# vibhaska/delta

Measured on AMD Instinct MI355X. Metric: log actions replayed/sec + achieved HBM GB/s, 1/2/4/8 GPU, 10M-file table, higher is better.
Workload: dtype u8/int64; 1 GPU; config 3: 10M-file checkpoint + 30 JSON commits, 16000032 actions -> 10000000 live files, 30% remove/re-add churn, retention cutoff; actions=16000032, json_bytes=1775145997, checkpoint_bytes=859787616, parallelism=single GPU

## Files before the change

### delta_amd/csrc/json_lane.h

```cpp
#pragma once
#include <cstdint>
#include <cstring>

#if defined(__HIPCC__)
#define JL_HD __host__ __device__ __forceinline__
#define JL_UNROLL _Pragma("unroll")
#else
#define JL_HD inline
#define JL_UNROLL
#endif

namespace dr {
namespace jl {

enum : uint8_t { K_NONE = 0, K_ADD = 1, K_REMOVE = 2, K_METADATA = 3, K_TXN = 4, K_PROTOCOL = 5, K_CDC = 6,
                 K_COMMITINFO = 7, K_ERROR = 15 };
enum : uint8_t { F_HAS_DELTS = 1, F_PATH_ESCAPED = 4, F_PATH_NULL = 8 };

struct LineOut {
  uint8_t kind;
  uint8_t flags;
  uint8_t hard;
  uint32_t path_off;
  uint32_t path_len;
  int64_t size;
  int64_t delts;
};

JL_HD uint32_t zbytes(uint32_t y) { return ~(((y & 0x7F7F7F7Fu) + 0x7F7F7F7Fu) | y | 0x7F7F7F7Fu); }
JL_HD uint32_t lt20(uint32_t x) { return ~((x | 0x80808080u) - 0x20202020u) & ~x & 0x80808080u; }
JL_HD uint32_t gather4(uint32_t m) {
  m >>= 7;
  m |= m >> 7;
  m |= m >> 14;
  return m & 0xFu;
}
JL_HD uint32_t prefix_xor16(uint32_t x) {
  x ^= x << 1;
  x ^= x << 2;
  x ^= x << 4;
  x ^= x << 8;
  return x & 0xFFFFu;
}

struct Win {
  uint32_t q, bs, st, sp, ctrl;
};

JL_HD uint32_t perm_b32(uint32_t s0, uint32_t s1, uint32_t sel) {
#if defined(__HIP_DEVICE_COMPILE__)
  return __builtin_amdgcn_perm(s0, s1, sel);
#else
  uint32_t r = 0;
  for (int k = 0; k < 4; ++k) {
    const uint32_t b = (sel >> (8 * k)) & 0xFFu;
    const uint32_t v = b < 4 ? (s1 >> (8 * b)) & 0xFFu : b < 8 ? (s0 >> (8 * (b - 4))) & 0xFFu : b == 0x0C ? 0u : 0xFFu;
    r |= v << (8 * k);
  }
  return r;
#endif
}
constexpr uint32_t CLS_LO0 = 0x40414048u, CLS_LO1 = 0x40404040u, CLS_LO2 = 0x44504040u, CLS_LO3 = 0x40404462u;
constexpr uint32_t CLS_HI0 = 0x10294040u, CLS_HI1 = 0x04000600u;
JL_HD uint32_t class_bytes(uint32_t x) {
  const uint32_t lo = x & 0x0F0F0F0Fu;
  const uint32_t sel = lo & 0x07070707u;
  const uint32_t a = perm_b32(CLS_LO1, CLS_LO0, sel), b = perm_b32(CLS_LO3, CLS_LO2, sel);
  const uint32_t m8 = perm_b32(0u, 0u, ((lo >> 3) & 0x01010101u) | 0x0C0C0C0Cu);
  const uint32_t tlo = (m8 & b) | (~m8 & a);
  const uint32_t thi = perm_b32(CLS_HI1, CLS_HI0, (x >> 4) & 0x07070707u);
  const uint32_t neg = perm_b32(0u, 0u, ((x >> 7) & 0x01010101u) | 0x0C0C0C0Cu);
  return tlo & thi & ~neg;
}
JL_HD uint32_t gather_bit(uint32_t r, int c) {
  uint32_t m = (r >> c) & 0x01010101u;
  m |= m >> 7;
  m |= m >> 14;
  return m & 0xFu;
}
JL_HD uint32_t delta_swap(uint32_t y, uint32_t delta, uint32_t mask) {
  const uint32_t t = (y ^ (y >> delta)) & mask;
  return y ^ t ^ (t << delta);
}

JL_HD void classify(const uint32_t w[4], Win& m) {
  uint32_t r[4], nib[4];
#if defined(__HIP_DEVICE_COMPILE__)
#pragma unroll
#endif
  for (int d = 0; d < 4; ++d) {
    r[d] = class_bytes(w[d]);
    nib[d] = (r[d] & 0x0F0F0F0Fu) | (((r[d] >> 2) | (r[d] >> 3)) & 0x04040404u);
  }
  uint32_t y0 = nib[0] | (nib[1] << 4), y1 = nib[2] | (nib[3] << 4);
  y0 = delta_swap(delta_swap(y0, 7, 0x00AA00AAu), 14, 0x0000CCCCu);
  y1 = delta_swap(delta_swap(y1, 7, 0x00AA00AAu), 14, 0x0000CCCCu);
  const uint32_t qb = perm_b32(y1, y0, 0x05010400u), ss = perm_b32(y1, y0, 0x07030602u);
  m.q = qb & 0xFFFFu;
  m.bs = qb >> 16;
  m.st = ss & 0xFFFFu;
  m.sp = ss >> 16;
  m.ctrl = 0;
  if ((r[0] | r[1] | r[2] | r[3]) & 0x40404040u)
    for (int d = 0; d < 4; ++d) m.ctrl |= gather_bit(r[d], 6) << (4 * d);
}

JL_HD uint32_t win_byte(const uint32_t w[4], uint32_t k) {
  const uint32_t d = k >> 2;
  const uint32_t x = d == 0 ? w[0] : d == 1 ? w[1] : d == 2 ? w[2] : w[3];
  return (x >> (8 * (k & 3))) & 0xFFu;
}

JL_HD uint32_t ctz32(uint32_t x) {
#if defined(__HIP_DEVICE_COMPILE__)
  return uint32_t(__builtin_ctz(x));
#else
  return uint32_t(__builtin_ctz(x));
#endif
}
JL_HD uint32_t popc32(uint32_t x) { return uint32_t(__builtin_popcount(x)); }

enum : uint8_t { SC_BAD = 0, SC_NULL, SC_TRUE, SC_FALSE, SC_INT, SC_NUM };

JL_HD bool key_eq(const uint8_t* s, uint32_t n, const char* k, uint32_t kn) {
  if (n != kn) return false;
  for (uint32_t i = 0; i < n; ++i)
    if (s[i] != uint8_t(k[i])) return false;
  return true;
}
JL_HD uint8_t action_key(const uint8_t* s, uint32_t n) {
  switch (n) {
    case 3:
      if (key_eq(s, n, "add", 3)) return K_ADD;
      if (key_eq(s, n, "txn", 3)) return K_TXN;
      if (key_eq(s, n, "cdc", 3)) return K_CDC;
      return 0;
    case 6: return key_eq(s, n, "remove", 6) ? K_REMOVE : 0;
    case 8:
      if (key_eq(s, n, "metaData", 8)) return K_METADATA;
      if (key_eq(s, n, "protocol", 8)) return K_PROTOCOL;
      return 0;
    case 10: return key_eq(s, n, "commitInfo", 10) ? K_COMMITINFO : 0;
    default: return 0;
  }
}
enum : uint8_t { FK_OTHER = 0, FK_PATH, FK_SIZE, FK_DELTS };
JL_HD uint8_t file_key(const uint8_t* s, uint32_t n) {
  if (n == 4) {
    if (key_eq(s, n, "path", 4)) return FK_PATH;
    if (key_eq(s, n, "size", 4)) return FK_SIZE;
    return FK_OTHER;
  }
  if (n == 17 && key_eq(s, n, "deletionTimestamp", 17)) return FK_DELTS;
  return FK_OTHER;
}

enum : uint32_t { T_OBJ_OPEN = 0, T_ARR_OPEN, T_OBJ_CLOSE, T_ARR_CLOSE, T_COLON, T_COMMA, T_STR_OPEN,
                  T_STR_CLOSE, T_STR_CLOSE_ESC, T_SCALAR, T_STRING, T_STRING_ESC, T_SCALAR_LONG = 13 };
enum : uint32_t { TF_COLON = 0x10u, TF_COMMA = 0x20u, TF_MASK = 0x30u };
constexpr uint32_t TOK_MAX_LINE = 65535;
constexpr uint32_t TOK_MAX_SCALAR = 4095;
constexpr uint32_t TOK_MAX_AUX = 1023;
// ... 433 lines not shown
    }
    d.state = S_AFTER;
  }
}

template <bool General>
JL_HD void dfa_token_own(const uint8_t* p, uint32_t tok, Dfa<General>& d) {
  const uint32_t cls = tok_cls(tok), off = tok_off(tok);
  const uint8_t stt = d.state;
  if (cls == T_STRING || cls == T_STRING_ESC) {
    if (dfa_str_open(off, d)) dfa_str_close(p, off + 1 + tok_aux(tok), cls == T_STRING_ESC, d);
    return;
  }
  if (cls == T_STR_OPEN) {
    dfa_str_open(off, d);
    return;
  }
  if (cls == T_STR_CLOSE || cls == T_STR_CLOSE_ESC) {
    dfa_str_close(p, off, cls == T_STR_CLOSE_ESC, d);
    return;
  }
  if (cls == T_SCALAR || cls == T_SCALAR_LONG) {
    if (!(stt == S_VALUE || stt == S_ARR_FIRST)) { d.status = ST_BAD; return; }
    const uint32_t L = cls == T_SCALAR ? tok_aux(tok) : tok_long_len(tok);
    int64_t v = 0;
    const uint8_t sc = scalar_fast(p + off, L, &v);
    if (sc == SC_BAD) { d.status = ST_BAD; return; }
    d.sc_checked += L;
    if (d.depth == 1) {
      if (sc == SC_NULL) {
        if (d.k1) d.present &= ~(1u << d.k1);
        if (d.k1 == K_ADD) d.fadd = FileObj{0, 0, 0, 0, F_PATH_NULL};
        if (d.k1 == K_REMOVE) d.frm = FileObj{0, 0, 0, 0, F_PATH_NULL};
      } else {
        if (d.k1 == K_ADD || d.k1 == K_REMOVE) { d.status = ST_BAD; return; }
        if (d.k1) d.present |= 1u << d.k1;
      }
    } else if (d.depth == 2 && d.in_file) {
      if (d.k2 == FK_PATH) {
        if (sc != SC_NULL) { d.status = ST_BAD; return; }
        d.cur.path_off = 0;
        d.cur.path_len = 0;
        d.cur.flags = uint8_t((d.cur.flags & ~F_PATH_ESCAPED) | F_PATH_NULL);
      } else if (d.k2 == FK_SIZE) {
        if (sc == SC_NULL) d.cur.size = 0;
        else if (sc == SC_INT) d.cur.size = v;
        else { d.status = ST_BAD; return; }
      } else if (d.k2 == FK_DELTS) {
        if (sc == SC_NULL) { d.cur.delts = 0; d.cur.flags &= ~F_HAS_DELTS; }
        else if (sc == SC_INT) { d.cur.delts = v; d.cur.flags |= F_HAS_DELTS; }
        else { d.status = ST_BAD; return; }
      }
    }
    d.state = S_AFTER;
    return;
  }
  if (cls == T_COLON) {
    if (stt != S_COLON) { d.status = ST_BAD; return; }
    d.state = S_VALUE;
    return;
  }
  if (cls == T_COMMA) {
    if (stt != S_AFTER || d.depth == 0) { d.status = ST_BAD; return; }
    d.state = d.is_arr(d.depth) ? S_VALUE : S_KEY;
    return;
  }
  if (cls == T_OBJ_OPEN || cls == T_ARR_OPEN) {
    const bool arr = cls == T_ARR_OPEN;
    if (!(stt == S_VALUE || stt == S_ARR_FIRST || (stt == S_START && !arr))) { d.status = ST_BAD; return; }
    if (d.depth == 2 && d.in_file && d.k2 != FK_OTHER) { d.status = ST_BAD; return; }
    if (d.depth == 1 && (d.k1 == K_ADD || d.k1 == K_REMOVE)) {
      if (arr) { d.status = ST_BAD; return; }
      d.in_file = true;
      d.k2 = FK_OTHER;
      d.cur = FileObj{0, 0, 0, 0, F_PATH_NULL};
    }
    if (d.depth >= 62) {
      if (!General) { d.status = ST_HARD; return; }
      if (d.depth + 1 >= GEN_MAX_DEPTH) { d.status = ST_BAD; return; }
    }
    ++d.depth;
    d.set_arr(d.depth, arr);
    d.state = arr ? S_ARR_FIRST : S_OBJ_FIRST;
    return;
  }
  {
    const bool arr = cls == T_ARR_CLOSE;
    if (d.depth == 0) { d.status = ST_BAD; return; }
    const bool top_arr = d.is_arr(d.depth);
    if (arr != top_arr || !(stt == S_AFTER || stt == (arr ? S_ARR_FIRST : S_OBJ_FIRST))) { d.status = ST_BAD; return; }
    if (d.depth == 2) {
      if (d.in_file) {
        const bool ad = d.k1 == K_ADD;
        d.fadd.path_off = ad ? d.cur.path_off : d.fadd.path_off;
        d.fadd.path_len = ad ? d.cur.path_len : d.fadd.path_len;
        d.fadd.size = ad ? d.cur.size : d.fadd.size;
        d.fadd.delts = ad ? d.cur.delts : d.fadd.delts;
        d.fadd.flags = ad ? d.cur.flags : d.fadd.flags;
        d.frm.path_off = ad ? d.frm.path_off : d.cur.path_off;
        d.frm.path_len = ad ? d.frm.path_len : d.cur.path_len;
        d.frm.size = ad ? d.frm.size : d.cur.size;
        d.frm.delts = ad ? d.frm.delts : d.cur.delts;
        d.frm.flags = ad ? d.frm.flags : d.cur.flags;
        d.in_file = false;
      }
      if (d.k1) d.present |= 1u << d.k1;
    }
    --d.depth;
    d.state = d.depth == 0 ? S_DONE : S_AFTER;
  }
}

template <bool General>
JL_HD void dfa_token(const uint8_t* p, uint32_t tok, Dfa<General>& d) {
  dfa_token_own<General>(p, tok, d);
  const uint32_t fl = tok_flags(tok);
  if (fl == 0 || d.status != ST_OK) return;
  const bool colon = (fl & TF_COLON) != 0;
  const bool ok = fl != TF_MASK && (colon ? d.state == S_COLON : (d.state == S_AFTER && d.depth != 0));
  if (!ok) { d.status = ST_BAD; return; }
  d.state = (colon || d.is_arr(d.depth)) ? S_VALUE : S_KEY;
}

template <bool General>
JL_HD void dfa_finish(const Tokenizer& tz, const Dfa<General>& d, LineOut& out) {
  out.kind = K_NONE;
  out.flags = 0;
  out.hard = 0;
  out.path_off = 0;
  out.path_len = 0;
  out.size = 0;
  out.delts = 0;
  if (tz.status == ST_HARD || d.status == ST_HARD) { out.hard = 1; return; }
  if (tz.status == ST_OK && d.status == ST_OK && d.state == S_START && tz.sc_bytes == 0) return;
  if (tz.status != ST_OK || d.status != ST_OK || d.state != S_DONE || tz.sc_bytes != d.sc_checked) {
    out.kind = K_ERROR;
    return;
  }
  const uint32_t pr = d.present;
  out.kind = (pr & (1u << K_ADD)) ? K_ADD : (pr & (1u << K_REMOVE)) ? K_REMOVE
           : (pr & (1u << K_METADATA)) ? K_METADATA : (pr & (1u << K_TXN)) ? K_TXN
           : (pr & (1u << K_PROTOCOL)) ? K_PROTOCOL : (pr & (1u << K_CDC)) ? K_CDC
           : (pr & (1u << K_COMMITINFO)) ? K_COMMITINFO : K_NONE;
  if (out.kind == K_ADD || out.kind == K_REMOVE) {
    const bool ad = out.kind == K_ADD;
    out.flags = ad ? d.fadd.flags : d.frm.flags;
    out.path_off = ad ? d.fadd.path_off : d.frm.path_off;
    out.path_len = ad ? d.fadd.path_len : d.frm.path_len;
    out.size = ad ? d.fadd.size : d.frm.size;
    out.delts = ad ? d.fadd.delts : d.frm.delts;
  }
}

template <bool General>
JL_HD void parse_line_t(const uint8_t* p, uint32_t n, LineOut& out) {
  Tokenizer tz;
  Dfa<General> d;
  if (n > TOK_MAX_LINE) {
    if (!General) { out = LineOut{0, 0, 1, 0, 0, 0, 0}; return; }
  }
  const uintptr_t pa = reinterpret_cast<uintptr_t>(p);
  const uint8_t* base = p - (pa & 15u);
  const uint32_t o0 = uint32_t(pa & 15);
  const uint32_t nwin = (o0 + n + 15) >> 4;
  auto step = [&](uint32_t t) {
    if (d.status == ST_OK) dfa_token<General>(p, t, d);
  };
  for (uint32_t j = 0; j < nwin && tz.status == ST_OK && d.status == ST_OK; ++j) {
    uint32_t w[4];
    load_window(base + 16u * j, w);
    tokenize_window<General>(p, n, w, int32_t(16u * j) - int32_t(o0), tz, step);
  }
  tokenize_end(n, tz, step);
  dfa_finish<General>(tz, d, out);
}

JL_HD void parse_line(const uint8_t* p, uint32_t n, LineOut& out) { parse_line_t<false>(p, n, out); }
JL_HD void parse_line_general(const uint8_t* p, uint32_t n, LineOut& out) { parse_line_t<true>(p, n, out); }

}
}
```

### delta_amd/csrc/k_json.hip

```cpp
#include <cstdlib>
#include <type_traits>

#include "dev_common.h"
#include "kernels.h"
#include "json_lane.h"
#include "canon.h"
#include "wave.h"
#include "ix_dev.h"

namespace dr {
namespace dev {

#ifdef DR_BOUNDS_CHECK
__device__ unsigned int dr_lds_bounds_hits;
#define DR_LDS_CHECK(ok, site, idx, lim)                                                                       \
  do {                                                                                                       \
    if (!(ok) && atomicAdd(&dr_lds_bounds_hits, 1u) < 32u)                                                   \
      printf("LDS-BOUNDS %s: index %llu, extent %llu (block %u thread %u)\n", site, (unsigned long long)(idx), \
             (unsigned long long)(lim), blockIdx.x, threadIdx.x);                                           \
  } while (0)
#else
#define DR_LDS_CHECK(ok, site, idx, lim) \
  do {                                   \
  } while (0)
// ... 14 lines not shown
template <typename Put>
__device__ __forceinline__ uint32_t block_newlines(const uint8_t* __restrict__ buf, uint64_t len, uint64_t blk,
                                                   Put put) {
  __shared__ uint32_t wsum[JSON_THREADS / 64];
  const uint32_t rel0 = threadIdx.x * JSON_BYTES_PER_THREAD;
  const uint64_t base = blk * JSON_BYTES_PER_BLOCK + rel0;
  uint32_t words[16];
  uint32_t c = 0;
  const bool full = base + JSON_BYTES_PER_THREAD <= len;
  if (full) {
    const uint4* p = reinterpret_cast<const uint4*>(buf + base);
#pragma unroll
    for (int i = 0; i < 4; ++i) {
      uint4 v = p[i];
      words[4 * i] = v.x; words[4 * i + 1] = v.y; words[4 * i + 2] = v.z; words[4 * i + 3] = v.w;
    }
#pragma unroll
    for (int i = 0; i < 16; ++i) c += count_nl_word(words[i]);
  } else {
    for (uint64_t i = base; i < len; ++i) c += buf[i] == '\n';
  }
  const int lane = threadIdx.x & 63, wv = threadIdx.x >> 6;
  uint32_t incl = c;
  for (int o = 1; o < 64; o <<= 1) {
    uint32_t t = __shfl_up(incl, o, 64);
    if (lane >= o) incl += t;
  }
  if (lane == 63) wsum[wv] = incl;
  __syncthreads();
  uint32_t woff = 0, total = 0;
  for (int i = 0; i < JSON_THREADS / 64; ++i) {
    woff += i < wv ? wsum[i] : 0u;
    total += wsum[i];
  }
  uint32_t r = woff + incl - c;
  if (full) {
#pragma unroll
    for (int i = 0; i < 16; ++i) {
      uint32_t t = nl_bytes(words[i]);
      while (t) {
        put(r++, rel0 + 4 * i + (__builtin_ctz(t) >> 3));
        t &= t - 1;
      }
    }
  } else {
    for (uint64_t i = base; i < len; ++i)
      if (buf[i] == '\n') put(r++, uint32_t(i - blk * JSON_BYTES_PER_BLOCK));
  }
  return total;
}

__global__ void __launch_bounds__(JSON_THREADS) k_json_index(const uint8_t* __restrict__ buf, uint64_t len,
                                                            uint32_t* __restrict__ block_counts,
                                                            uint16_t* __restrict__ slots) {
  uint16_t* slot = slots + uint64_t(blockIdx.x) * JSON_SLOT;
  const uint32_t total = block_newlines(buf, len, blockIdx.x, [&](uint32_t r, uint32_t pos) {
    if (r < uint32_t(JSON_SLOT)) slot[r] = uint16_t(pos);
  });
  if (threadIdx.x == 0) block_counts[blockIdx.x] = total;
}

__global__ void __launch_bounds__(JSON_THREADS) k_json_index1(const uint8_t* __restrict__ buf, uint64_t len,
                                                             uint64_t* __restrict__ nl, uint64_t* __restrict__ off2,
                                                             uint64_t* __restrict__ zero, uint32_t nzero) {
  if (threadIdx.x < nzero) zero[threadIdx.x] = 0;
  const uint32_t total = block_newlines(buf, len, 0, [&](uint32_t r, uint32_t pos) { nl[r] = pos; });
  if (threadIdx.x == 0) {
    off2[0] = 0;
    off2[1] = total;
  }
}

__global__ void __launch_bounds__(JSON_THREADS) k_json_place(const uint8_t* __restrict__ buf, uint64_t len,
                                                            const uint32_t* __restrict__ block_counts,
                                                            const uint64_t* __restrict__ block_off,
                                                            const uint16_t* __restrict__ slots,
                                                            uint64_t* __restrict__ nl) {
  const uint32_t cnt = block_counts[blockIdx.x];
  const uint64_t base = uint64_t(blockIdx.x) * JSON_BYTES_PER_BLOCK;
  uint64_t* out = nl + block_off[blockIdx.x];
  if (cnt <= uint32_t(JSON_SLOT)) {
    const uint16_t* slot = slots + uint64_t(blockIdx.x) * JSON_SLOT;
    for (uint32_t k = threadIdx.x; k < cnt; k += JSON_THREADS) out[k] = base + slot[k];
  } else {
    block_newlines(buf, len, blockIdx.x, [&](uint32_t r, uint32_t pos) { out[r] = base + pos; });
  }
}

constexpr int JL_T = 64;

__device__ __forceinline__ void emit_line(const JsonParseArgs& a, uint64_t line, uint64_t b, uint32_t n,
                                          const uint8_t* lp, const uint8_t* gp, const jl::LineOut& o) {
  const uint64_t idx = a.base + line;
  uint8_t flags = 0;
  uint64_t key = 0, path = 0;
  uint32_t plen = 0;
  int64_t size = 0, delts = 0;
  const uint8_t kind = o.kind;
  if (kind == K_ADD || kind == K_REMOVE) {
    flags = o.flags;
    path = reinterpret_cast<uint64_t>(gp + o.path_off);
    plen = o.path_len;
    size = o.size;
    delts = o.delts;
    if (!(flags & F_PATH_NULL)) {
      if ((flags & F_PATH_ESCAPED) || path_is_special(lp + o.path_off, plen)) {
        flags |= F_SPECIAL_PATH;
        atomicAdd(reinterpret_cast<unsigned long long*>(a.special_count), 1ull);
        atomicAdd(reinterpret_cast<unsigned long long*>(a.special_bytes), (unsigned long long)(plen + 8));
      } else {
        key = path_key(lp + o.path_off, plen);
      }
    } else {
      path = 0;
      plen = 0;
    }
  } else if (kind == K_METADATA || kind == K_TXN || kind == K_PROTOCOL) {
    const unsigned long long slot = atomicAdd(reinterpret_cast<unsigned long long*>(a.nonfile_count), 1ull);
    if (slot < a.nonfile_cap) {
      a.nonfile_idx[2 * slot] = line;
      a.nonfile_idx[2 * slot + 1] = b;
    }
  } else if (kind == K_ERROR) {
    atomicAdd(reinterpret_cast<unsigned long long*>(a.error_count), 1ull);
  }
  a.kind[idx] = kind;
  a.flags[idx] = flags;
  a.key[idx] = key;
  a.path_ptr[idx] = path;
  a.path_len[idx] = plen;
  if (a.path_ref) a.path_ref[idx] = pack_ref(path, plen);
  a.size[idx] = size;
  a.delts[idx] = delts;
  a.src_off[idx] = b;
  a.src_len[idx] = n;
}

#ifndef DR_JL_TOKCAP
#define DR_JL_TOKCAP 40
#endif
constexpr int JL_TOKCAP = DR_JL_TOKCAP;
#ifndef DR_JL_FLUSH
#define DR_JL_FLUSH (DR_JL_TOKCAP - 18)
#endif
static_assert(DR_JL_FLUSH >= 0 && DR_JL_FLUSH + 18 <= DR_JL_TOKCAP, "a window's tokens must fit behind the flush mark");
constexpr int JL_FLUSH = DR_JL_FLUSH;

#ifndef DR_JL_BATCH
#define DR_JL_BATCH 2
#endif
#ifndef DR_JL_WAVES
#define DR_JL_WAVES 1
#endif
constexpr uint32_t JL_SMALL_LINES = 256;
constexpr uint32_t JL_STAGE_BYTES = 24u * 1024u;

template <bool InlineHard = false>
__device__ __forceinline__ void walk_line(const JsonParseArgs& a, uint32_t* tokbuf, uint32_t lane, uint64_t line,
                                          bool live, uint64_t b, uint32_t n, const uint8_t* p) {
  jl::Tokenizer tz;
  jl::Dfa<false> d;
  if (!live) tz.status = jl::ST_BAD;
  else if (n > jl::TOK_MAX_LINE) tz.status = jl::ST_HARD;
  const uint32_t o0 = uint32_t(b & 15);
  const uint8_t* base = p - o0;
  const uint32_t nwin = tz.status == jl::ST_OK ? (o0 + n + 15) >> 4 : 0;
  uint32_t nt = 0;
#if DR_JL_BATCH > 1
  uint4 batch[DR_JL_BATCH];
#endif
  auto push = [&](uint32_t t) {
    DR_LDS_CHECK(nt < uint32_t(JL_TOKCAP), "walk_line tokbuf", nt, JL_TOKCAP);
    tokbuf[nt * JL_T + lane] = t;
    ++nt;
  };
  for (uint32_t j = 0;; ++j) {
    if (j < nwin && tz.status == jl::ST_OK) {
      uint32_t w[4];
#if DR_JL_BATCH > 1
      if (j % DR_JL_BATCH == 0) {
        const uint4* q = reinterpret_cast<const uint4*>(base + 16u * j);
#pragma unroll
        for (int k = 0; k < DR_JL_BATCH; ++k) batch[k] = j + k < nwin ? q[k] : make_uint4(0, 0, 0, 0);
      }
      uint4 v0 = batch[0];
#pragma unroll
      for (int k = 1; k < DR_JL_BATCH; ++k)
        if (j % DR_JL_BATCH == uint32_t(k)) v0 = batch[k];
      w[0] = v0.x; w[1] = v0.y; w[2] = v0.z; w[3] = v0.w;
#else
      jl::load_window(base + 16u * j, w);
#endif
      jl::tokenize_window<false>(p, n, w, int32_t(16u * j) - int32_t(o0), tz, push);
      if (j + 1 == nwin) jl::tokenize_end(n, tz, push);
    }
    const bool more = j + 1 < nwin && tz.status == jl::ST_OK;
    const bool anymore = __ballot(more) != 0ull;
    if (!anymore || __ballot(nt > uint32_t(JL_FLUSH)) != 0ull) {
      uint32_t mx = nt;
      for (int o = 32; o > 0; o >>= 1) mx = max(mx, uint32_t(__shfl_xor(int(mx), o, 64)));
#if !defined(DR_JL_EXP)
      for (uint32_t t = 0; t < mx; ++t)
        if (t < nt && d.status == jl::ST_OK) jl::dfa_token<false>(p, tokbuf[t * JL_T + lane], d);
#endif
      nt = 0;
    }
    if (!anymore) break;
  }
  if (!live) return;
  jl::LineOut o;
  jl::dfa_finish<false>(tz, d, o);
  if (o.hard) {
    if constexpr (InlineHard) {
      const uint8_t* gp = a.buf + b;
      jl::parse_line_general(gp, n, o);
      emit_line(a, line, b, n, gp, gp, o);
    } else {
      const unsigned long long k = atomicAdd(a.hard_count, 1ull);
      a.hard_idx[k] = line;
    }
    return;
  }
  emit_line(a, line, b, n, p, a.buf + b, o);
}

constexpr uint32_t T_NL = 12;
constexpr uint32_t TAPE_CAP = 4096;

constexpr uint64_t STRUCT_CLS = (uint64_t(jl::T_COLON) << 40) | (uint64_t(jl::T_OBJ_OPEN) << 44) |
                                (uint64_t(jl::T_COMMA) << 48) | (uint64_t(jl::T_OBJ_CLOSE) << 52);

__device__ __forceinline__ uint32_t escape16(uint32_t bs, uint32_t cin, uint32_t* cout) {
  const uint32_t bsn = bs & ~cin;
  const uint32_t follows = ((bsn << 1) | cin) & 0xFFFFu;
  const uint32_t odd_starts = bsn & ~0x5555u & ~follows;
  const uint32_t sum = odd_starts + bsn;
  *cout = (sum >> 16) & 1u;
  return (0x5555u ^ ((sum << 1) & 0xFFFFu)) & follows;
}

__device__ __forceinline__ uint64_t lanes_below() { return (1ull << wv::lane_id()) - 1ull; }

__device__ __forceinline__ void wave_sync() {
  __builtin_amdgcn_fence(__ATOMIC_RELEASE, "wavefront");
  __builtin_amdgcn_wave_barrier();
  __builtin_amdgcn_fence(__ATOMIC_ACQUIRE, "wavefront");
}

__device__ __forceinline__ int32_t from_lower(bool has, int32_t v, int32_t dflt) {
  constexpr uint32_t NONE = 0x80000000u;
  uint32_t x = has ? uint32_t(v) : NONE;
  x = wv::scan_incl(x, NONE, [](uint32_t e, uint32_t l) { return l == NONE ? e : l; });
  x = wv::shr1(x, NONE);
  return x == NONE ? dflt : int32_t(x);
}

template <uint32_t TCap, uint32_t NL, uint32_t SW>
__device__ __forceinline__ bool build_tape(const uint4* stage, uint32_t rb, uint32_t R, uint32_t nlines, uint32_t* tape,
                           uint16_t* nltok, uint8_t* tline, unsigned long long* phase = nullptr) {
  const uint32_t lane = wv::lane_id();
  DR_LDS_CHECK(uint64_t(rb) + R + 48 <= uint64_t(SW) * 16, "build_tape region", uint64_t(rb) + R + 48, SW * 16);
  if (uint64_t(rb) + R + 48 > uint64_t(SW) * 16) return false;
  const uint32_t a0 = rb & ~15u;
  const uint32_t skew = rb - a0;
  const uint32_t total = skew + R;
  const uint32_t nsteps = (total + 1023u) >> 10;
  uint32_t esc_c = 0, instr_c = 0, sc_c = 0, tbase = 0, nlc = 0;
  int32_t open_c = -1, bs_c = -1;
  for (uint32_t s = 0; s < nsteps; ++s) {
    const uint64_t ts0 = phase ? __builtin_amdgcn_s_memtime() : 0;
    const uint32_t wpos = (s << 10) + (lane << 4);
    const int32_t lo = int32_t(wpos) - int32_t(skew);
    DR_LDS_CHECK(wpos >= total || ((a0 + wpos) >> 4) < SW, "build_tape stage", (a0 + wpos) >> 4, SW);
    const uint4 v = stage[min((a0 + wpos) >> 4, SW - 1)];
    const uint32_t keep = wpos < total ? ~0u : 0u;
    const uint32_t w[4] = {v.x & keep, v.y & keep, v.z & keep, v.w & keep};
    const uint32_t vlo = lo < 0 ? (0xFFFFu << uint32_t(min(-lo, 16))) & 0xFFFFu : 0xFFFFu;
    const int32_t rem = int32_t(R) - lo;
    const uint32_t vhi = rem >= 16 ? 0xFFFFu : rem <= 0 ? 0u : (1u << uint32_t(rem)) - 1u;
    const uint32_t valid = vlo & vhi;
    jl::Win m;
    jl::classify(w, m);
    m.q &= valid; m.bs &= valid; m.st &= valid; m.sp &= valid; m.ctrl &= valid;
    uint32_t nl = 0;
#pragma unroll
    for (int d = 0; d < 4; ++d) nl |= jl::gather4(jl::zbytes(w[d] ^ 0x0a0a0a0au)) << (4 * d);
    nl &= valid;
    uint32_t c0;
    escape16(m.bs, 0u, &c0);
    const bool allbs = m.bs == 0xFFFFu;
    const uint32_t cin = uint32_t(from_lower(!allbs, int32_t(c0), int32_t(esc_c)));
    uint32_t cout;
    const uint32_t escaped = escape16(m.bs, cin, &cout);
    esc_c = uint32_t(__builtin_amdgcn_readlane(int(allbs ? cin : cout), 63));
    const uint32_t quote = m.q & ~escaped;
    const unsigned long long par = __ballot(__builtin_popcount(quote) & 1);
    const uint32_t sin = instr_c ^ uint32_t(__popcll(par & lanes_below()) & 1);
    const uint32_t instr = jl::prefix_xor16(quote) ^ (sin ? 0xFFFFu : 0u);
    instr_c ^= uint32_t(__popcll(par) & 1);
    bool bad = (m.ctrl & ~(nl & ~instr)) != 0 || (m.sp & ~instr) != 0;
    uint32_t oddesc = escaped & ~(m.q | m.bs) & valid;
    while (oddesc) {
      const uint32_t k = jl::ctz32(oddesc);
      oddesc &= oddesc - 1;
      const uint32_t c = jl::win_byte(w, k);
      bad |= !(c == '/' || c == 'b' || c == 'f' || c == 'n' || c == 'r' || c == 't');
    }
    const uint32_t st = m.st & ~instr;
    const uint32_t sc = valid & ~instr & ~quote & ~st & ~m.sp & ~m.ctrl;
    const uint32_t sc_prev = wv::shr1(sc >> 15, sc_c) & 1u;
    const uint32_t sc_begin = sc & ~(((sc << 1) | sc_prev) & 0xFFFFu);
    sc_c = uint32_t(__builtin_amdgcn_readlane(int(sc >> 15), 63)) & 1u;
    const uint32_t open = quote & instr, close = quote & ~instr;
    const uint32_t bsin = m.bs & instr;
    const int32_t last_open = open ? lo + 31 - __builtin_clz(open) : -1;
    const int32_t last_bs = bsin ? lo + 31 - __builtin_clz(bsin) : -1;
    const int32_t open_in = from_lower(open != 0, last_open, open_c);
    const int32_t bs_in = from_lower(bsin != 0, last_bs, bs_c);
    open_c = __builtin_amdgcn_readlane(open ? last_open : open_in, 63);
    bs_c = __builtin_amdgcn_readlane(bsin ? last_bs : bs_in, 63);
    const uint32_t tm = st | close | sc_begin | nl;
    const uint32_t cnt = uint32_t(__builtin_popcount(tm)) | (uint32_t(__builtin_popcount(nl)) << 16);
    const uint32_t incl = wv::scan_incl(cnt, 0u, [](uint32_t e, uint32_t l) { return e + l; });
    const uint32_t tot = uint32_t(__builtin_amdgcn_readlane(int(incl), 63));
    if (__ballot(bad)) return false;
    if (tbase + (tot & 0xFFFFu) > TCap || nlc + (tot >> 16) > NL) return false;
    uint32_t idx = tbase + ((incl - cnt) & 0xFFFFu);
    uint32_t nlr = nlc + ((incl - cnt) >> 16);
    bool longstr = false;
    const uint64_t ts1 = phase ? __builtin_amdgcn_s_memtime() : 0;
    uint32_t t = tm;
    const uint64_t wlo = uint64_t(w[0]) | (uint64_t(w[1]) << 32), whi = uint64_t(w[2]) | (uint64_t(w[3]) << 32);
    while (t) {
      const uint32_t k = jl::ctz32(t);
      t &= t - 1;
      const uint32_t bit = 1u << k, below = bit - 1u;
      const uint32_t pos = uint32_t(lo + int32_t(k));
      const uint32_t ob = open & below, bb = bsin & below;
      const int32_t op = ob ? lo + 31 - __builtin_clz(ob) : open_in;
      const int32_t lb = bb ? lo + 31 - __builtin_clz(bb) : bs_in;
      const uint32_t blen = pos - uint32_t(op) - 1u;
      const uint32_t c = uint32_t(((k & 8u) ? whi : wlo) >> ((k & 7u) * 8u)) & 0xFFu;
      const uint32_t lo4 = c & 15u;
      const uint32_t scls = uint32_t((STRUCT_CLS >> (4u * lo4)) & 15u) + (((0x2800u >> lo4) & ~(c >> 5)) & 1u);
      const bool isclose = (close & bit) != 0;
      longstr |= isclose & (blen >= 4096u);
      const uint32_t stok = (uint32_t(op) << 16) | ((blen & 0xFFFu) << 4) | (lb > op ? jl::T_STRING_ESC : jl::T_STRING);
      const uint32_t otok = (pos << 16) | ((st & bit) ? scls : (sc_begin & bit) ? jl::T_SCALAR : T_NL);
      DR_LDS_CHECK(idx < TCap, "build_tape tape", idx, TCap);
      DR_LDS_CHECK(nlr < NL || !(nl & bit), "build_tape nltok", nlr, NL);
      tline[idx] = uint8_t(nlr);
      const bool isnl = (nl & bit) != 0;
      nltok[isnl ? nlr : NL] = uint16_t(idx);
      nlr += isnl ? 1u : 0u;
      tape[idx++] = isclose ? stok : otok;
    }
    if (phase && lane == 0) {
      atomicAdd(&phase[6], (unsigned long long)(ts1 - ts0));
      atomicAdd(&phase[7], (unsigned long long)(__builtin_amdgcn_s_memtime() - ts1));
    }
    if (__ballot(longstr)) return false;
    tbase += tot & 0xFFFFu;
    nlc += tot >> 16;
  }
// ... 70 lines not shown
       : (L == 5 && w0[0] == 0x736C6166u && (w0[1] & 0xFFu) == 0x65u) ? jl::SC_FALSE
       : (isint && fits) ? jl::SC_INT : jl::SC_BAD;
}

template <uint32_t TCap, uint32_t NL>
__device__ __forceinline__ void tape_lines(const JsonParseArgs& a, uint64_t line0, uint32_t nlines, const uint8_t* sp,
                                           uint32_t sp_ext, uint64_t gb, const uint32_t* tape, const uint16_t* nltok,
                                           const uint8_t* tline, TapeAgg<NL>& g) {
  (void)sp_ext;
  const uint32_t lane = wv::lane_id();
  const uint64_t tw0 = a.phase ? __builtin_amdgcn_s_memtime() : 0;
  if (lane < NL) {
#pragma unroll
    for (int k = 0; k < 8; ++k) {
      g.mem[lane][k] = -1;
      g.fld[lane][k >> 2][k & 3] = -1;
    }
    g.defer[lane] = 0;
  }
  wave_sync();
  const uint32_t ntok = uint32_t(nltok[nlines - 1]) + 1u;
  int32_t dcarry = 0, ocarry = -1;
  uint32_t tcarry = 0, ptail1 = T_NL, ptail2 = T_NL;
  for (uint32_t r0 = 0; r0 < ntok; r0 += JL_T) {
    const uint32_t i = r0 + lane;
    const bool in = i < ntok;
    const uint32_t tk = tape[min(i, TCap - 1)], nx = tape[min(i + 1, TCap - 1)];
    const uint32_t tl = tline[min(i, TCap - 1)];
    const uint32_t tok = in ? tk : 15u;
    const uint32_t nxt = i + 1 < ntok ? nx : tok;
    const uint32_t line = in ? tl : 0u;
    const uint32_t ptok = wv::shr1(tok, ptail1), pptok = wv::shr1(ptok, ptail2);
    ptail1 = wv::last_uniform(tok);
    ptail2 = wv::last_uniform(ptok);
    uint32_t sw[5], kw[5];
    DR_LDS_CHECK(!in || (tok >> 16) + 24u <= sp_ext, "tape_lines token bytes", (tok >> 16) + 24u, sp_ext);
    DR_LDS_CHECK(!in || (pptok >> 16) + 25u <= sp_ext, "tape_lines key bytes", (pptok >> 16) + 25u, sp_ext);
    DR_LDS_CHECK(!in || line < NL, "tape_lines line", line, NL);
    lds20(sp + (tok >> 16), sw);
    lds20(sp + (pptok >> 16) + 1u, kw);
    const uint32_t cls = tok & 0xFu;
    const uint32_t pc0 = ptok & 0xFu;
    const bool first = pc0 == T_NL;
    const uint32_t ppc0 = pptok & 0xFu;
    const int32_t delta = cls <= jl::T_ARR_OPEN ? 1 : (cls == jl::T_OBJ_CLOSE || cls == jl::T_ARR_CLOSE) ? -1 : 0;
    const uint32_t kk = key_kinds(kw, (pptok >> 4) & 0xFFFu);
    const uint32_t k1 = kk & 0xFu, k2 = kk >> 4;
    uint32_t sg = (first ? 0x80000000u : 0u) | (uint32_t(delta) & 0x7FFFFFFFu);
    sg = wv::scan_incl(sg, 0u, [](uint32_t e, uint32_t l) {
      return (l & 0x80000000u) ? l : ((e & 0x80000000u) | ((e + l) & 0x7FFFFFFFu));
    });
    int32_t v = int32_t(sg << 1) >> 1;
    if (!(sg & 0x80000000u)) v += dcarry;
    dcarry = __builtin_amdgcn_readlane(v, 63);
    const int32_t D = v - delta;
    const bool opens = delta > 0;
    uint32_t x = opens && v <= int32_t(TW_LEVELS) ? ((1u << v) | (uint32_t(cls == jl::T_ARR_OPEN) << (8 + v))) : 0u;
    x = type_combine(tcarry, wv::scan_incl(x, 0u, type_combine));
    tcarry = wv::last_uniform(x);
    const bool m2open = opens && v == 2 && pc0 == jl::T_COLON;
    int32_t o2 = int32_t(wv::scan_incl(m2open ? (i << 3) | k1 : 0xFFFFFFFFu, 0xFFFFFFFFu,
                                       [](uint32_t e, uint32_t l) { return uint32_t(max(int32_t(e), int32_t(l))); }));
    o2 = max(o2, ocarry);
    ocarry = __builtin_amdgcn_readlane(o2, 63);
    const bool lvl = D >= 1 && D <= int32_t(TW_LEVELS) && ((x >> D) & 1u);
    const bool ctx_arr = lvl && ((x >> (8 + D)) & 1u), ctx_obj = lvl && !ctx_arr;
    const uint32_t ppc = (first || ppc0 == T_NL) ? 15u : ppc0;
    const bool is_str = cls == jl::T_STRING || cls == jl::T_STRING_ESC;
    const bool is_sc = cls == jl::T_SCALAR;
    const bool pstr = pc0 == jl::T_STRING || pc0 == jl::T_STRING_ESC;
    const bool prev_key = pstr && (ppc == jl::T_OBJ_OPEN || (ppc == jl::T_COMMA && ctx_obj));
    const bool prev_vend = pc0 == jl::T_SCALAR || pc0 == jl::T_OBJ_CLOSE || pc0 == jl::T_ARR_CLOSE || (pstr && !prev_key);
    const bool value_pos = pc0 == jl::T_COLON || (ctx_arr && (pc0 == jl::T_ARR_OPEN || pc0 == jl::T_COMMA));
    const bool cur_key = is_str && (pc0 == jl::T_OBJ_OPEN || (pc0 == jl::T_COMMA && ctx_obj));
    int64_t sv;
    const uint32_t L = (nxt >> 16) - (tok >> 16);
    const uint8_t sc = scalar_tape(sw, L, &sv);
    const bool is_nl = cls == T_NL;
    const bool inner = !is_nl & !first & (D >= 1);
    const bool okv = (is_nl & (D == 0)) | (!is_nl & first & (cls == jl::T_OBJ_OPEN)) |
                     (inner & ((opens & value_pos & (v <= int32_t(TW_LEVELS))) |
                               (is_sc & value_pos & (sc != jl::SC_BAD)) |
                               (is_str & ((cur_key & !((cls == jl::T_STRING_ESC) & (D <= 2))) | value_pos)) |
                               ((cls == jl::T_COLON) & prev_key) | ((cls == jl::T_COMMA) & prev_vend) |
                               ((cls == jl::T_OBJ_CLOSE) & ctx_obj & ((pc0 == jl::T_OBJ_OPEN) | prev_vend)) |
                               ((cls == jl::T_ARR_CLOSE) & ctx_arr & ((pc0 == jl::T_ARR_OPEN) | prev_vend))));
    const bool member = in & !first & (pc0 == jl::T_COLON);
    const bool nonnull = !(is_sc & (sc == jl::SC_NULL));
    const int32_t rec = int32_t(2u * i) + (nonnull ? 1 : 0);
    const uint32_t ek1 = uint32_t(o2) & (o2 >= 0 ? 7u : 0u);
    const bool file1 = (k1 == jl::K_ADD) | (k1 == jl::K_REMOVE), efile = (ek1 == jl::K_ADD) | (ek1 == jl::K_REMOVE);
    const bool m1 = member & (D == 1) & (k1 != 0);
    const bool mf = member & (D == 2) & efile & (k2 != jl::FK_OTHER);
    const bool bad1 = m1 & file1 & nonnull & (cls != jl::T_OBJ_OPEN);
    const bool path_ok = is_str | !nonnull, num_ok = is_sc & ((sc == jl::SC_NULL) | (sc == jl::SC_INT));
    const bool badf = mf & !((k2 == jl::FK_PATH) ? path_ok : num_ok);
    if (m1) atomicMax(&g.mem[line][k1], rec);
    if (mf) atomicMax(&g.fld[line][ek1 == jl::K_REMOVE ? 1 : 0][k2], rec);
    if (in & !(okv & !bad1 & !badf)) g.defer[line] = 1u;
    if (a.phase && r0 == 0 && lane == 0) atomicAdd(&a.phase[5], (unsigned long long)(__builtin_amdgcn_s_memtime() - tw0));
  }
  wave_sync();
  if (a.phase && lane == 0) atomicAdd(&a.phase[3], (unsigned long long)(__builtin_amdgcn_s_memtime() - tw0));
  if (lane >= nlines) return;
  const uint64_t line = line0 + lane;
  const uint32_t te = nltok[lane];
  const uint32_t ts = lane ? uint32_t(nltok[lane - 1]) + 1u : 0u;
  DR_LDS_CHECK(te < TCap && ts <= TCap, "tape_lines line tokens", te, TCap);
  const uint32_t ls = lane ? (tape[ts - 1] >> 16) + 1u : 0u;
  const uint32_t n = (tape[te] >> 16) - ls;
  if (g.defer[lane]) {
    const unsigned long long k = atomicAdd(a.hard_count, 1ull);
    a.hard_idx[k] = line;
    return;
  }
  jl::LineOut o{};
  o.kind = jl::K_NONE;
  const uint8_t order[7] = {jl::K_ADD, jl::K_REMOVE, jl::K_METADATA, jl::K_TXN, jl::K_PROTOCOL, jl::K_CDC, jl::K_COMMITINFO};
#pragma unroll
  for (int k = 6; k >= 0; --k)
    if (g.mem[lane][order[k]] >= 0 && (g.mem[lane][order[k]] & 1)) o.kind = order[k];
  if (o.kind == jl::K_ADD || o.kind == jl::K_REMOVE) {
    const int32_t m = g.mem[lane][o.kind] >> 1;
    const int32_t* fl = g.fld[lane][o.kind == jl::K_REMOVE ? 1 : 0];
    o.flags = jl::F_PATH_NULL;
    const int32_t tp = fl[jl::FK_PATH], tz = fl[jl::FK_SIZE], td = fl[jl::FK_DELTS];
    if (tp >= 0 && (tp >> 1) > m && (tp & 1)) {
      DR_LDS_CHECK(uint32_t(tp >> 1) < TCap, "tape_lines path token", tp >> 1, TCap);
      const uint32_t t = tape[tp >> 1];
      o.path_off = (t >> 16) + 1u - ls;
      o.path_len = (t >> 4) & 0xFFFu;
      o.flags = (t & 0xFu) == jl::T_STRING_ESC ? jl::F_PATH_ESCAPED : 0;
    }
    const bool hz = tz >= 0 && (tz >> 1) > m && (tz & 1), hd = td >= 0 && (td >> 1) > m && (td & 1);
    const uint32_t iz = hz ? uint32_t(tz >> 1) : 0u, id = hd ? uint32_t(td >> 1) : 0u;
    DR_LDS_CHECK(iz + 1 < TCap && id + 1 < TCap, "tape_lines scalar tokens", max(iz, id) + 1, TCap);
    const uint32_t az = tape[iz], bz = tape[min(iz + 1, TCap - 1)], ad = tape[id], bd = tape[min(id + 1, TCap - 1)];
    DR_LDS_CHECK((az >> 16) + 24u <= sp_ext && (ad >> 16) + 24u <= sp_ext, "tape_lines scalar bytes",
                 max(az >> 16, ad >> 16) + 24u, sp_ext);
    uint32_t wz[5], wd[5];
    lds20(sp + (az >> 16), wz);
    lds20(sp + (ad >> 16), wd);
    int64_t vz, vd;
    (void)scalar_tape(wz, (bz >> 16) - (az >> 16), &vz);
    (void)scalar_tape(wd, (bd >> 16) - (ad >> 16), &vd);
    o.size = hz ? vz : 0;
    o.delts = hd ? vd : 0;
    if (hd) o.flags |= jl::F_HAS_DELTS;
  }
  emit_line(a, line, gb + ls, n, sp + ls, a.buf + gb + ls, o);
}

template <bool Stage>
__global__ void __launch_bounds__(JL_T, DR_JL_WAVES) k_json_lines(JsonParseArgs a) {
  __shared__ uint32_t tokbuf[Stage ? 1 : JL_TOKCAP * JL_T];
  __shared__ uint4 stage[Stage ? JL_STAGE_BYTES / 16 : 1];
  __shared__ uint32_t tape[Stage ? TAPE_CAP : 1];
  __shared__ uint16_t nltok[Stage ? JL_T + 1 : 1];
  __shared__ uint8_t tline[Stage ? TAPE_CAP : 1];
  __shared__ std::conditional_t<Stage, TapeAgg<JL_T>, uint32_t> agg;
  const uint32_t lane = threadIdx.x;
  const uint64_t line = uint64_t(blockIdx.x) * JL_T + lane;
  const bool live = line < a.nlines;
  if constexpr (Stage) {
    uint64_t tp0 = a.phase ? __builtin_amdgcn_s_memtime() : 0;
    auto phase = [&](int k) {
      if (!a.phase) return;
      const uint64_t t = __builtin_amdgcn_s_memtime();
      if (lane == 0) atomicAdd(&a.phase[k], (unsigned long long)(t - tp0));
      tp0 = t;
    };
    if (a.zero) {
      if (lane < a.nzero) a.zero[lane] = 0;
      const uint32_t len = uint32_t(a.buf_len);
      const uint4* src = reinterpret_cast<const uint4*>(a.buf);
      const uint32_t nq = ((len + 15u) >> 4) + 3u;
      DR_LDS_CHECK(nq <= JL_STAGE_BYTES / 16, "k_json_lines fused stage", nq, JL_STAGE_BYTES / 16);
      for (uint32_t k = lane; k < min(nq, JL_STAGE_BYTES / 16); k += JL_T) stage[k] = src[k];
      __threadfence();
      __syncthreads();
      phase(0);
      const uint32_t nw = uint32_t(a.nlines);
      const bool taped = build_tape<TAPE_CAP, JL_T, JL_STAGE_BYTES / 16>(stage, 0u, len, nw, tape, nltok, tline, a.phase);
      phase(1);
      __syncthreads();
      if (taped) {
        DR_LDS_CHECK(lane >= nw || lane < JL_T, "k_json_lines nltok", lane, JL_T);
        if (lane < nw) a.nl_out[lane] = tape[nltok[lane]] >> 16;
        if (lane == 0) {
          a.off2[0] = 0;
          a.off2[1] = nw;
        }
        tape_lines<TAPE_CAP, JL_T>(a, 0, nw, reinterpret_cast<const uint8_t*>(stage), JL_STAGE_BYTES, 0, tape, nltok, tline,
                                   agg);
        phase(2);
        if (a.phase && lane == 0) atomicAdd(&a.phase[4], 1ull);
        return;
      }
      uint32_t base = 0;
      for (uint32_t s0 = 0; s0 < len; s0 += 16u * JL_T) {
        const uint32_t wpos = s0 + 16u * lane;
        DR_LDS_CHECK(wpos >= len || (wpos >> 4) < JL_STAGE_BYTES / 16, "k_json_lines stage", wpos >> 4,
                     JL_STAGE_BYTES / 16);
        const uint4 v = stage[min(wpos >> 4, JL_STAGE_BYTES / 16 - 1)];
        const uint32_t w[4] = {v.x, v.y, v.z, v.w};
        uint32_t m = 0;
#pragma unroll
        for (int d = 0; d < 4; ++d) m |= jl::gather4(jl::zbytes(w[d] ^ 0x0a0a0a0au)) << (4 * d);
        const int32_t rem = int32_t(len) - int32_t(wpos);
        m &= rem >= 16 ? 0xFFFFu : rem <= 0 ? 0u : (1u << uint32_t(rem)) - 1u;
        const uint32_t c = __builtin_popcount(m);
        const uint32_t incl = wv::scan_incl(c, 0u, [](uint32_t e, uint32_t l) { return e + l; });
        uint32_t r = base + incl - c;
        while (m) {
          a.nl_out[r++] = wpos + jl::ctz32(m);
          m &= m - 1;
        }
        base += wv::last_uniform(incl);
      }
      if (lane == 0) {
        a.off2[0] = 0;
        a.off2[1] = base;
        atomicAdd(a.hard_count, (unsigned long long)nw);
      }
      if (lane < nw) a.hard_idx[lane] = lane;
      return;
    }
    const uint64_t first = uint64_t(blockIdx.x) * JL_T;
    const uint64_t last = min(first + JL_T, a.nlines) - 1;
    const uint64_t r0 = (first == 0 ? 0 : a.nl[first - 1] + 1) & ~uint64_t(15);
    const uint64_t r1 = (a.nl[last] + 16) & ~uint64_t(15);
    if (r1 - r0 + 48 <= JL_STAGE_BYTES) {
      const uint4* src = reinterpret_cast<const uint4*>(a.buf + r0);
      const uint32_t nq = uint32_t((r1 - r0) >> 4) + 3;
      for (uint32_t k = lane; k < nq; k += JL_T) stage[k] = src[k];
      __syncthreads();
      phase(0);
      const uint32_t nw = uint32_t(last - first + 1);
      const uint64_t rb = first == 0 ? 0 : a.nl[first - 1] + 1;
      const bool taped = build_tape<TAPE_CAP, JL_T, JL_STAGE_BYTES / 16>(stage, uint32_t(rb - r0), uint32_t(a.nl[last] + 1 - rb), nw,
                                                                       tape, nltok, tline, a.phase);
      phase(1);
      if (taped) {
        __syncthreads();
        tape_lines<TAPE_CAP, JL_T>(a, first, nw, reinterpret_cast<const uint8_t*>(stage) + (rb - r0),
                                   JL_STAGE_BYTES - uint32_t(rb - r0), rb, tape, nltok, tline, agg);
        phase(2);
        if (a.phase && lane == 0) atomicAdd(&a.phase[4], 1ull);
        return;
      }
    }
    if (live) {
      const unsigned long long k = atomicAdd(a.hard_count, 1ull);
      a.hard_idx[k] = line;
    }
    return;
  }
  const uint64_t b = !live ? 0 : line == 0 ? 0 : a.nl[line - 1] + 1;
  const uint32_t n = live ? uint32_t(a.nl[line] - b) : 0;
  walk_line(a, tokbuf, lane, line, live, b, n, a.buf + b);
}

__global__ void __launch_bounds__(64) k_json_hard(JsonParseArgs a) {
  const uint64_t cnt = *a.hard_count;
  for (uint64_t k = uint64_t(blockIdx.x) * blockDim.x + threadIdx.x; k < cnt; k += uint64_t(gridDim.x) * blockDim.x) {
    const uint64_t line = a.hard_idx[k];
    const uint64_t b = line == 0 ? 0 : a.nl[line - 1] + 1;
    const uint32_t n = uint32_t(a.nl[line] - b);
    const uint8_t* gp = a.buf + b;
    jl::LineOut o;
    jl::parse_line_general(gp, n, o);
    emit_line(a, line, b, n, gp, gp, o);
  }
}

__device__ __forceinline__ void tail_post_body(const JsonParseArgs& a, const CanonArgs& c) {
  const uint64_t cnt = __hip_atomic_load(a.hard_count, __ATOMIC_RELAXED, __HIP_MEMORY_SCOPE_AGENT);
  const uint64_t nsp0 = __hip_atomic_load(a.special_count, __ATOMIC_RELAXED, __HIP_MEMORY_SCOPE_AGENT);
  for (uint64_t k = threadIdx.x; k < cnt; k += blockDim.x) {
    const uint64_t line = a.hard_idx[k];
    DR_LDS_CHECK(line < a.nlines, "tail_post deferred line (global)", line, a.nlines);
#ifdef DR_BOUNDS_CHECK
    if (line >= a.nlines) continue;
#endif
    const uint64_t b = line == 0 ? 0 : a.nl[line - 1] + 1;
    DR_LDS_CHECK(b <= a.nl[line] && a.nl[line] < a.buf_len, "tail_post line bytes (global)", a.nl[line], a.buf_len);
#ifdef DR_BOUNDS_CHECK
    if (!(b <= a.nl[line] && a.nl[line] < a.buf_len)) continue;
#endif
    const uint32_t n = uint32_t(a.nl[line] - b);
    const uint8_t* gp = a.buf + b;
    jl::LineOut o;
    jl::parse_line_general(gp, n, o);
    emit_line(a, line, b, n, gp, gp, o);
  }
  if (!cnt && !nsp0) return;
  __threadfence_block();
  __syncthreads();
  for (uint64_t i = threadIdx.x; i < c.n; i += blockDim.x) canon_one(c, i);
}

__global__ void __launch_bounds__(256) k_tail_post(JsonParseArgs a, CanonArgs c) { tail_post_body(a, c); }

__device__ __forceinline__ void apply_small_body(const JsonParseArgs& a, const CanonArgs& c, const AppendArgs& p,
                                                 const IndexArgs& x, bool ctr_set) {
  const uint32_t t = threadIdx.x;
  __shared__ unsigned long long sums[6];
// ... 226 lines not shown
```

Baseline: 1.838 billion actions/s.

## Add fixed-shape writer-line matcher to skip DFA for add/remove lines

Adds a fast path that matches tokenized add/remove lines against the fixed member order emitted by the standard writer, encoded as packed 64-bit shape words. When a line fits entirely in one token flush and matches, the general DFA pass is skipped; otherwise the DFA runs as before. It also raises the launch-bounds waves hint for the non-staged kernel, which caps register use to allow more occupancy. The risks are extra divergence and code size from the matcher, and possible spills under the tighter register budget.

```diff
diff --git a/delta_amd/csrc/json_lane.h b/delta_amd/csrc/json_lane.h
--- a/delta_amd/csrc/json_lane.h
+++ b/delta_amd/csrc/json_lane.h
@@ -5,9 +5,11 @@
 #if defined(__HIPCC__)
 #define JL_HD __host__ __device__ __forceinline__
 #define JL_UNROLL _Pragma("unroll")
+#define JL_NOUNROLL _Pragma("nounroll")
 #else
 #define JL_HD inline
 #define JL_UNROLL
+#define JL_NOUNROLL
 #endif
 
 namespace dr {
@@ -747,6 +749,119 @@
   }
 }
 
+enum : uint8_t { WV_STRING = 0, WV_SCALAR = 1, WV_PVALS = 2 };
+struct WMember {
+  uint8_t klen, fk, val, opt;
+};
+constexpr WMember W_ADD[] = {{4, FK_PATH, WV_STRING, 0},   {15, FK_OTHER, WV_PVALS, 0},  {4, FK_SIZE, WV_SCALAR, 0},
+                             {16, FK_OTHER, WV_SCALAR, 0}, {10, FK_OTHER, WV_SCALAR, 0}, {5, FK_OTHER, WV_STRING, 1}};
+constexpr WMember W_REMOVE[] = {{4, FK_PATH, WV_STRING, 0},   {17, FK_DELTS, WV_SCALAR, 0}, {10, FK_OTHER, WV_SCALAR, 0},
+                                {20, FK_OTHER, WV_SCALAR, 1}, {15, FK_OTHER, WV_PVALS, 0},  {4, FK_SIZE, WV_SCALAR, 0}};
+constexpr uint32_t W_BITS = 10;
+template <int N>
+constexpr uint64_t wshape(const WMember (&m)[N]) {
+  static_assert(N * W_BITS <= 64, "a shape is one 64-bit word");
+  uint64_t s = 0;
+  for (int i = N - 1; i >= 0; --i)
+    s = (s << W_BITS) | uint64_t(m[i].klen | (m[i].fk << 5) | (m[i].val << 7) | (m[i].opt << 9));
+  return s;
+}
+constexpr uint64_t W_ADD_SHAPE = wshape(W_ADD), W_REMOVE_SHAPE = wshape(W_REMOVE);
+
+JL_HD bool match_writer_line(const uint8_t* p, uint32_t n, const uint32_t* tok, uint32_t stride, uint32_t nt,
+                             const Tokenizer& tz, LineOut& out) {
+  (void)n;
+  if (tz.status != ST_OK) return false;
+  uint32_t t = 0;
+  auto next = [&]() -> uint32_t { return t < nt ? tok[(t++) * stride] : TOK_NONE; };
+  constexpr uint32_t CF = 0x3Fu;
+  if ((next() & CF) != T_OBJ_OPEN) return false;
+  const uint32_t ak = next();
+  if ((ak & CF) != (T_STRING | TF_COLON)) return false;
+  const uint8_t kind = action_key_w(p + tok_off(ak) + 1, tok_aux(ak));
+  if (kind != K_ADD && kind != K_REMOVE) return false;
+  if ((next() & CF) != T_OBJ_OPEN) return false;
+  uint32_t checked = 0;
+  uint32_t path_off = 0, path_len = 0;
+  uint8_t flags = F_PATH_NULL;
+  int64_t size = 0, delts = 0;
+  bool comma = true;
+JL_NOUNROLL
+  for (uint64_t shape = kind == K_ADD ? W_ADD_SHAPE : W_REMOVE_SHAPE; shape; shape >>= W_BITS) {
+    const uint32_t m = uint32_t(shape) & ((1u << W_BITS) - 1u);
+    const uint32_t klen = m & 31u, fk = (m >> 5) & 3u, val = (m >> 7) & 3u;
+    if (!comma) {
+      if (!(m >> 9)) return false;
+      break;
+    }
+    const uint32_t k = next();
+    if ((k & CF) != (T_STRING | TF_COLON) || tok_aux(k) != klen) return false;
+    if (file_key_w(p + tok_off(k) + 1, klen) != fk) return false;
+    uint32_t v = next();
+    const uint32_t cls = tok_cls(v);
+    if (val == WV_STRING) {
+      if (cls != T_STRING && cls != T_STRING_ESC) return false;
+      if (fk == FK_PATH) {
+        path_off = tok_off(v) + 1;
+        path_len = tok_aux(v);
+        flags = cls == T_STRING_ESC ? F_PATH_ESCAPED : 0;
+      }
+    } else if (val == WV_SCALAR) {
+      if (cls != T_SCALAR) return false;
+      int64_t x = 0;
+      const uint8_t sc = scalar_fast(p + tok_off(v), tok_aux(v), &x);
+      if (sc == SC_BAD) return false;
+      checked += tok_aux(v);
+      if (fk != FK_OTHER) {
+        if (sc != SC_INT && sc != SC_NULL) return false;
+        if (fk == FK_SIZE) size = x;
+        else {
+          delts = x;
+          if (sc == SC_INT) flags |= F_HAS_DELTS;
+        }
+      }
+    } else {
+      if ((v & CF) != T_OBJ_OPEN) return false;
+      bool need_key = false;
+      for (;;) {
+        v = next();
+        if ((v & CF) != (T_STRING | TF_COLON)) break;
+        const uint32_t pv = next();
+        const uint32_t pc = tok_cls(pv), pf = pv & TF_MASK;
+        if (pc == T_SCALAR) {
+          uint32_t w[5];
+          load20(p + tok_off(pv), 4, w);
+          if (tok_aux(pv) != 4 || w[0] != 0x6C6C756Eu) return false;
+          checked += 4;
+        } else if (pc != T_STRING && pc != T_STRING_ESC) {
+          return false;
+        }
+        if (pf & TF_COLON) return false;
+        need_key = pf != 0;
+        if (!need_key) {
+          v = next();
+          break;
+        }
+      }
+      if (need_key || tok_cls(v) != T_OBJ_CLOSE) return false;
+    }
+    const uint32_t vf = v & TF_MASK;
+    if (vf & TF_COLON) return false;
+    comma = vf != 0;
+  }
+  if (comma) return false;
+  if ((next() & CF) != T_OBJ_CLOSE || (next() & CF) != T_OBJ_CLOSE || t != nt) return false;
+  if (tz.sc_bytes != checked) return false;
+  out.kind = kind;
+  out.flags = flags;
+  out.hard = 0;
+  out.path_off = path_off;
+  out.path_len = path_len;
+  out.size = size;
+  out.delts = delts;
+  return true;
+}
+
 template <bool General>
 JL_HD void parse_line_t(const uint8_t* p, uint32_t n, LineOut& out) {
   Tokenizer tz;
diff --git a/delta_amd/csrc/k_json.hip b/delta_amd/csrc/k_json.hip
--- a/delta_amd/csrc/k_json.hip
+++ b/delta_amd/csrc/k_json.hip
@@ -190,6 +190,9 @@
 #ifndef DR_JL_WAVES
 #define DR_JL_WAVES 1
 #endif
+#ifndef DR_JL_BULK_WAVES
+#define DR_JL_BULK_WAVES 4
+#endif
 constexpr uint32_t JL_SMALL_LINES = 256;
 constexpr uint32_t JL_STAGE_BYTES = 24u * 1024u;
 
@@ -197,7 +200,7 @@
 __device__ __forceinline__ void walk_line(const JsonParseArgs& a, uint32_t* tokbuf, uint32_t lane, uint64_t line,
                                           bool live, uint64_t b, uint32_t n, const uint8_t* p) {
   jl::Tokenizer tz;
-  jl::Dfa<false> d;
+  jl::LineOut o;
   if (!live) tz.status = jl::ST_BAD;
   else if (n > jl::TOK_MAX_LINE) tz.status = jl::ST_HARD;
   const uint32_t o0 = uint32_t(b & 15);
@@ -212,6 +215,9 @@
     tokbuf[nt * JL_T + lane] = t;
     ++nt;
   };
+  jl::Dfa<false> d;
+  bool flushed = false;
+  bool matched = false;
   for (uint32_t j = 0;; ++j) {
     if (j < nwin && tz.status == jl::ST_OK) {
       uint32_t w[4];
@@ -235,19 +241,27 @@
     const bool more = j + 1 < nwin && tz.status == jl::ST_OK;
     const bool anymore = __ballot(more) != 0ull;
     if (!anymore || __ballot(nt > uint32_t(JL_FLUSH)) != 0ull) {
-      uint32_t mx = nt;
-      for (int o = 32; o > 0; o >>= 1) mx = max(mx, uint32_t(__shfl_xor(int(mx), o, 64)));
 #if !defined(DR_JL_EXP)
-      for (uint32_t t = 0; t < mx; ++t)
-        if (t < nt && d.status == jl::ST_OK) jl::dfa_token<false>(p, tokbuf[t * JL_T + lane], d);
+      bool need = true;
+      if (!anymore && !flushed) {
+        matched = live && jl::match_writer_line(p, n, tokbuf + lane, JL_T, nt, tz, o);
+        need = live && !matched;
+        d = jl::Dfa<false>();
+      }
+      if (__ballot(need) != 0ull) {
+        uint32_t mx = need ? nt : 0u;
+        for (int s = 32; s > 0; s >>= 1) mx = max(mx, uint32_t(__shfl_xor(int(mx), s, 64)));
+        for (uint32_t t = 0; t < mx; ++t)
+          if (need && t < nt && d.status == jl::ST_OK) jl::dfa_token<false>(p, tokbuf[t * JL_T + lane], d);
+      }
 #endif
       nt = 0;
+      flushed = true;
     }
     if (!anymore) break;
   }
   if (!live) return;
-  jl::LineOut o;
-  jl::dfa_finish<false>(tz, d, o);
+  if (!matched) jl::dfa_finish<false>(tz, d, o);
   if (o.hard) {
     if constexpr (InlineHard) {
       const uint8_t* gp = a.buf + b;
@@ -624,7 +638,7 @@
 }
 
 template <bool Stage>
-__global__ void __launch_bounds__(JL_T, DR_JL_WAVES) k_json_lines(JsonParseArgs a) {
+__global__ void __launch_bounds__(JL_T, Stage ? DR_JL_WAVES : DR_JL_BULK_WAVES) k_json_lines(JsonParseArgs a) {
   __shared__ uint32_t tokbuf[Stage ? 1 : JL_TOKCAP * JL_T];
   __shared__ uint4 stage[Stage ? JL_STAGE_BYTES / 16 : 1];
   __shared__ uint32_t tape[Stage ? TAPE_CAP : 1];
```

New measurement: 1.894 billion actions/s (median of 6 runs). 3.1% higher.
